# EI-CoreBioinformatics/portcullis

Measured on AMD Instinct MI355X. Metric: junc_reads_per_sec, higher is better.
Workload: dtype int32; 1 GPU; BASELINE configs[2]: synthetic 199999998 paired-end 150-bp reads, 25 contigs of GRCh38 lengths (3088286401 bp), 249999 junctions, orientation FR; reads_total=199999998, junctions_total=249999, contigs=25, reads_rank0=199999998, pairs_rank0=66692850

## Files before the change

portcullis_amd/csrc/pjb_api.hip:

```cpp
#include "pjb_host.hip.h"
#include "pjb_kernels.hip.h"

static int slot_init(pjb_ctx *c, int k);
static void aux_streams(pjb_ctx *c) {
    if (!c->stream3) (void)hipStreamCreateWithFlags(&c->stream3, hipStreamNonBlocking);
    if (!c->stream4) (void)hipStreamCreateWithFlags(&c->stream4, hipStreamNonBlocking);
}

extern "C" {

namespace {
std::mutex g_host_mu;
std::map<void *, size_t> g_host_registered;
}
void *pjb_host_alloc(size_t bytes) {
    if (bytes >= ((size_t)8 << 20)) {
        const size_t huge = (size_t)2 << 20, len = (bytes + huge - 1) & ~(huge - 1);
        void *p = mmap(nullptr, len, PROT_READ | PROT_WRITE, MAP_PRIVATE | MAP_ANONYMOUS, -1, 0);
        if (p != MAP_FAILED) {
            (void)madvise(p, len, MADV_HUGEPAGE);
            const size_t nt = std::min<size_t>(4, len >> 24);
            auto touch = [&](size_t t) {
                const size_t per = ((len / std::max<size_t>(nt, 1)) + huge - 1) & ~(huge - 1), a = std::min(len, per * t), b = std::min(len, a + per);
                for (size_t o = a; o < b; o += 4096) ((volatile uint8_t *)p)[o] = 0;
// ... 157 lines not shown
    extra_clear(c);
    for (auto &kv : c->filter_keys)
        if (kv.second.first) (void)hipFree(kv.second.first);
    c->filter_keys.clear();
    for (auto &g : c->contigs) free_contig(g);
    for (auto &b : c->genome_pool) release(b);
    c->genome_pool.clear();
    for (auto &sl : c->slab_pool)
        if (sl.p) (void)hipFree(sl.p);
    if (c->rows_pinned) (void)hipHostFree(c->rows_pinned);
    if (c->rows_table) (void)hipFree(c->rows_table);
    bam_stage_clear(c);
    for (int k = 0; k < PJB_MAX_QUEUED; k++) {
        CtlSlot &S = c->sl[k];
        if (S.pub) (void)hipHostFree(S.pub);
        if (S.batches_pinned) (void)hipHostFree(S.batches_pinned);
        for (auto &ev : S.ev)
            if (ev) (void)hipEventDestroy(ev);
        if (S.ev_rows) (void)hipEventDestroy(S.ev_rows);
        if (S.ev_done) (void)hipEventDestroy(S.ev_done);
        Buf *sb[] = {&S.x_q, &S.x_spos, &S.x_send, &S.x_gapoff, &S.x_zlist, &S.x_scnt, &S.x_codes, &S.cstats, &S.err, &S.gencount, &S.batches, &S.rows, &S.tile_cnt, &S.tile_stats, &S.splidx, &S.splpoff, &S.splrec, &S.tile_soff, &S.chunk_tile, &S.scan_parts, &S.members, &S.okey, &S.g,
                     &S.rec, &S.jidbam, &S.jkey, &S.total, &S.bitmap, &S.wrank, &S.pagecnt, &S.pagerank, &S.ends, &S.firstid,
                     &S.key[0], &S.key[1], &S.idx[0], &S.idx[1], &S.hist, &S.hist_scan, &S.hist_part, &S.bintotal, &S.scan_tiles, &S.jid, &S.seg, &S.runfirst,
                     &S.runstart, &S.ent, &S.entsum, &S.frag, &S.fragj, &S.masks, &S.acc, &S.ancl, &S.ancr, &S.genlist};
        for (Buf *b : sb) release(*b);
        hipEvent_t evs[] = {S.ev_k1, S.ev_xk1, S.ev_fork, S.ev_join, S.ev_fork2, S.ev_join2};
        for (hipEvent_t e : evs)
            if (e) (void)hipEventDestroy(e);
        if (S.main) (void)hipStreamDestroy(S.main);
        if (S.side) (void)hipStreamDestroy(S.side);
    }
    if (c->mirror_hdr) (void)hipHostFree(c->mirror_hdr);
    for (int k = 0; k < 2; k++) {
        if (c->stage[k]) (void)hipHostFree(c->stage[k]);
        if (c->stage_ev[k]) (void)hipEventDestroy(c->stage_ev[k]);
    }
    Buf *all[] = {&c->b_cursor, &c->b_scan_tiles, &c->b_hasx, &c->b_xtotal, &c->b_fasta_raw, &c->b_inf_comp, &c->b_inf_out, &c->b_inf_blocks, &c->b_inf_status, &c->b_inf_scratch, &c->b_inf_bitmap,
                  &c->b_bam_seg, &c->b_bam_rec, &c->b_bam_ctl, &c->f_pos, &c->f_cigoff, &c->f_cigar, &c->f_codes, &c->g_rows, &c->g_models, &c->g_refs,
                  &c->g_out, &c->g_bad,
                  &c->x_pos, &c->x_endx, &c->x_q, &c->x_prefq, &c->x_ce, &c->x_bound, &c->x_de, &c->x_dropped, &c->x_zlist, &c->x_cnt,
                  &c->x_tabk, &c->x_tabc, &c->x_rs, &c->x_re, &c->x_rr, &c->x_tileoff, &c->x_xrall, &c->x_tab,
                  &c->b_dfl_in, &c->b_dfl_sym, &c->b_dfl_slots, &c->b_dfl_size, &c->b_dfl_off, &c->b_dfl_packed};
    for (Buf *b : all) release(*b);
    for (auto &ch : c->xarena.chunks) (void)hipFree(ch.p);
    if (c->xrows_pinned) (void)hipHostFree(c->xrows_pinned);
    for (auto &pool : c->pools)
        for (auto &ev : pool.ev) (void)hipEventDestroy(ev);
// ... 590 lines not shown
        LAUNCH(c, "k4b_generic", k4b_generic, dim3(gen_grid), dim3(256), (const u64 *)S.genlist.p, (const u32 *)d_gen_cnt, gen_cap, (const u64 *)pr.key,
               pr.rec, (const u32 *)S.jidbam.p, kf, (const DevBatch *)S.batches.p, (int)batches.size(), (const int32_t *)S.ancl.p, (const int32_t *)S.ancr.p,
               GT, any_x ? 1 : 0, any_x ? 0 : 1, d_err, (const ContigStats *)d_cs, pack_nn, (const u32 *)S.splidx.p, (const uint4 *)S.splrec.p);
        return PJB_OK;
    };
    auto fork_k4b = [&]() -> int {
        if (!c->side_stream) return launch_k4b();
        HIP_TRY(c, hipEventRecord(S.ev_fork, st));
        HIP_TRY(c, hipStreamWaitEvent(S.side, S.ev_fork, 0));
        c->stream = S.side;
        f.forked = true;
        const int rc2 = launch_k4b();
        c->stream = st;
        if (rc2) return rc2;
        HIP_TRY(c, hipEventRecord(S.ev_join, S.side));
        return PJB_OK;
    };

    int sort_bits = kf.total_bits;
    const u32 rs_tiles = std::max<u32>(1, (PL + RS_TILE - 1) / RS_TILE);
    int n_pass = 1;
    std::vector<int> pass_bits;
    bool first_hist_done = false;
    auto plan_passes = [&]() -> int {
        n_pass = (sort_bits + c->radix_max_bits - 1) / c->radix_max_bits;
        if (n_pass < 1) n_pass = 1;
        pass_bits.assign((size_t)n_pass, sort_bits / n_pass);
        for (int p = 0; p < sort_bits % n_pass; p++) pass_bits[(size_t)p]++;
        const int dbits = pass_bits[0];
        int rc2;
        if ((rc2 = ensure(c, S.hist, (size_t)rs_tiles * (1u << dbits) * 4))) return rc2;
        if ((rc2 = ensure(c, S.hist_scan, (size_t)rs_tiles * (1u << dbits) * 4))) return rc2;
        if ((rc2 = ensure(c, S.bintotal, (size_t)4 << dbits))) return rc2;
        if ((rc2 = ensure(c, S.hist_part, (size_t)((rs_tiles + RSP_TILES - 1) / RSP_TILES) * (1u << dbits) * 4))) return rc2;
        return PJB_OK;
    };
    if (lim.dense) {
        const u32 cand_blocks = std::min<u32>(pair_blocks, 1024u);
        const u64 *okey = (const u64 *)pr.key;
        u64 *cand = (u64 *)S.key[1].p;
        const u32 n_pages = (u32)((n_words + ((size_t)1 << KD_PAGE_SHIFT) - 1) >> KD_PAGE_SHIFT);
        if ((rc = run_scan(c, "kd_rank", ArrU32Fn{(const u32 *)S.pagecnt.p}, ExclusiveU32Sink{(u32 *)S.pagerank.p}, (u64)n_pages, (u64 *)S.total.p)))
            return rc;
        LAUNCH(c, "kd_rank_pages", kd_rank_pages, dim3((n_pages + 3) / 4), dim3(256), (const u64 *)S.bitmap.p, (const u32 *)S.pagecnt.p, (const u32 *)S.pagerank.p,
               (u32 *)S.wrank.p, n_pages, (u32)n_words);
        u32 *cand_rank = (u32 *)S.idx[1].p;
        LAUNCH(c, "kd_ends", kd_ends, dim3(cand_blocks), dim3(256), (const u64 *)cand, kf, (const u64 *)S.bitmap.p, (const u32 *)S.wrank.p, JL,
               (u32 *)S.ends.p, cand_rank, d_cs);
        if ((rc = run_scan(c, "kd_first", EndsCountFn{(const u32 *)S.ends.p}, FirstIdSink{(u32 *)S.firstid.p, (int32_t *)S.ancl.p, (int32_t *)S.ancr.p},
                           (u64)JL, (u64 *)S.total.p)))
            return rc;
        LAUNCH(c, "kd_table", kd_table, dim3(cand_blocks), dim3(256), (const u64 *)cand, (const u64 *)S.ent.p, (const u32 *)cand_rank, kf, JL,
               (const u32 *)S.ends.p, (const u32 *)S.firstid.p, (const u64 *)S.total.p, (u64 *)S.jkey.p, (int32_t *)S.ancl.p, (int32_t *)S.ancr.p, d_cs,
               (const u32 *)d_gen_cnt, gen_cap, SL);
        sort_bits = std::max(1, bits_of((uint64_t)SL));
        if ((rc = plan_passes())) return rc;
        LAUNCH(c, "kd_assign", kd_assign, dim3(rs_tiles), dim3(256), okey, d_P, kf, (const u64 *)S.bitmap.p, (const u32 *)S.wrank.p,
               (const u32 *)S.ends.p, (const u32 *)S.firstid.p, JL, (const u64 *)S.total.p, (u32 *)S.jidbam.p, (u32 *)S.acc.p, (const u64 *)S.jkey.p,
               (const int32_t *)S.ancl.p, (const int32_t *)S.ancr.p, d_err, d_cs, pass_bits[0], (u32 *)S.hist.p);
        first_hist_done = true;
        if ((rc = fork_k4b())) return rc;
        LAUNCH(c, "kd_reset", kd_reset, dim3(cand_blocks), dim3(256), (const u64 *)cand, (const u32 *)cand_rank, kf, JL, (const ContigStats *)d_cs,
               (u64 *)S.bitmap.p, (u32 *)S.ends.p, (u32 *)S.pagecnt.p);
        S.dense_at_rest = true;
    } else if ((rc = plan_passes()))
        return rc;
    int cur = 0, shift = 0;
    auto sort_pass = [&](auto key_tag, const void *kin_v, void *kout_v, const u32 *vin, u32 *vout, int bits) -> int {
        using K = decltype(key_tag);
        const K *kin = (const K *)kin_v;
        K *kout = (K *)kout_v;
        if (!(shift == 0 && first_hist_done))
            LAUNCH(c, "rs_hist", rs_hist<K>, dim3(rs_tiles), dim3(256), kin, d_P, shift, bits, (u32 *)S.hist.p, rs_tiles);
        {
            const u32 nb = 1u << bits, n_panels = (rs_tiles + RSP_TILES - 1) / RSP_TILES;
            LAUNCH(c, "rs_panel_sums", rs_panel_sums, dim3(n_panels, (nb + 255) / 256), dim3(256), (const u32 *)S.hist.p, rs_tiles, nb, (u32 *)S.hist_part.p);
            LAUNCH(c, "rs_panel_scan", rs_panel_scan, dim3(n_panels, (nb + 255) / 256), dim3(256), (const u32 *)S.hist.p, (const u32 *)S.hist_part.p, rs_tiles, nb,
                   (u32 *)S.hist_scan.p, (u32 *)S.bintotal.p);
        }
#define RS_SCATTER(B)                                                                                                                          \
    LAUNCH_LDS(c, "rs_scatter", (rs_scatter<B, K>), dim3(rs_tiles), dim3(256), rs_scatter_lds_bytes(bits, sizeof(K)), kin, vin, kout, vout, d_P, \
               shift, bits, (const u32 *)S.hist_scan.p, (const u32 *)S.bintotal.p, rs_tiles)
        switch (bits) {
        case 9: RS_SCATTER(9); break;
        case 10: RS_SCATTER(10); break;
        case 11: RS_SCATTER(11); break;
        default: RS_SCATTER(0); break;
        }
#undef RS_SCATTER
        return PJB_OK;
    };
    for (int p = 0; p < n_pass; p++) {
        const int bits = pass_bits[(size_t)p];
        if (bits <= 0) break;
        const u32 *vin = p == 0 ? nullptr : (const u32 *)S.idx[cur].p;
        u32 *vout = (u32 *)S.idx[cur ^ 1].p;
        if (lim.dense) rc = sort_pass((u32)0, p == 0 ? S.jidbam.p : S.key[cur].p, S.key[cur ^ 1].p, vin, vout, bits);
        else rc = sort_pass((u64)0, p == 0 ? S.okey.p : S.key[cur].p, S.key[cur ^ 1].p, vin, vout, bits);
        if (rc) return rc;
        cur ^= 1;
        shift += bits;
    }
    f.n_pass = n_pass;
    const u32 *sidx = (const u32 *)S.idx[cur].p;
    f.sidx = sidx;
    const u32 *jid_sorted = lim.dense ? (const u32 *)S.key[cur].p : (const u32 *)S.jid.p;
    f.jid_sorted = jid_sorted;
    STAGE_EVENT(2);
    if ((rc = ensure(c, S.entsum, (size_t)JL * 8 + 16))) return rc;
    const u32 n_slices_lim = (PL + 63) / 64 + 1;
    const hipStream_t tl = st;
    auto entropy_kernels = [&]() -> int {
        LAUNCH(c, "k5_entropy_sum", k5_entropy_sum, dim3(std::max<u32>(1, (JL + 15) / 16)), dim3(256), (const u32 *)S.seg.p, (const u32 *)S.runfirst.p,
               (const u32 *)S.runstart.p, d_J, (double *)S.entsum.p);
        return PJB_OK;
    };
    bool entropy_forked = false;
    auto fork_entropy = [&]() -> int {
        if (!c->side_stream) return entropy_kernels();
        HIP_TRY(c, hipEventRecord(S.ev_fork2, st));
        HIP_TRY(c, hipStreamWaitEvent(S.side, S.ev_fork2, 0));
        c->stream = S.side;
        entropy_forked = true;
        const int rc2 = entropy_kernels();
// ... 168 lines not shown
            f.m_reads[m] += b.n;
            if (oc.last_known[k]) {
                prev_pos = oc.last_pos[k];
                prev_ptr = nullptr;
            } else
                prev_ptr = b.pos + (b.n - 1);
            b.member = (int32_t)m;
            f.batches.push_back(b);
            f.batch_member.push_back((int)m);
        }
    }
    f.tile_lo[f.tids.size()] = f.n_tiles;
    f.vlen = f.tids.size() > 1 ? at : c->ref_len[(size_t)f.tid];
    f.empty = f.batches.empty();
    ContigLimits &lim = f.lim;
    const u64 guess = std::min<u64>(0xffffff00ull, (u64)f.n_reads * 5 / 8 + 4096);
    lim.pair_limit = (u32)std::max<u64>(guess, 4096);
    lim.junc_limit = std::max<u32>(std::max<u32>(lim.pair_limit / 32, 4096), 2 * c->junc_seen * (u32)std::max<size_t>(1, f.tids.size() > 1 ? 2 : 1));
    if (!genomes_ok) lim.pair_limit = 0;
    lim.kf.raw = 0;
    lim.kf.lbits = std::max(1, c->lbits_seen);
    lim.kf.total_bits = lim.kf.lbits + std::max(1, bits_of((uint64_t)std::max<int64_t>(f.vlen, 1)));
    lim.dense = c->dense_ids;
    lim.sort_limit = c->junc_per_read > 0 ? std::min<u32>(lim.junc_limit, std::max<u32>(c->sort_floor, (u32)std::min<double>(4.0e9, 2.0 * c->junc_per_read * (double)f.n_reads + 64.0))) : 0u;
}

static int slot_init(pjb_ctx *c, int k) {
    CtlSlot &S = c->sl[k];
    if (S.ev_done) return PJB_OK;
    for (auto &ev : S.ev) HIP_TRY(c, hipEventCreate(&ev));
    HIP_TRY(c, hipEventCreateWithFlags(&S.ev_rows, hipEventDisableTiming));
    HIP_TRY(c, hipEventCreateWithFlags(&S.ev_done, hipEventDisableTiming));
    HIP_TRY(c, hipEventCreateWithFlags(&S.ev_k1, hipEventDisableTiming));
    HIP_TRY(c, hipEventCreateWithFlags(&S.ev_xk1, hipEventDisableTiming));
    HIP_TRY(c, hipEventCreateWithFlags(&S.ev_fork, hipEventDisableTiming));
    HIP_TRY(c, hipEventCreateWithFlags(&S.ev_join, hipEventDisableTiming));
    HIP_TRY(c, hipEventCreateWithFlags(&S.ev_fork2, hipEventDisableTiming));
    HIP_TRY(c, hipEventCreateWithFlags(&S.ev_join2, hipEventDisableTiming));
    HIP_TRY(c, hipStreamCreateWithFlags(&S.main, hipStreamNonBlocking));
    HIP_TRY(c, hipStreamCreateWithFlags(&S.side, hipStreamNonBlocking));
    return PJB_OK;
}

static int queue_chain(pjb_ctx *c, Flight &f) {
    int rc = queue_contig(c, f);
    if (!rc && c->extra) rc = extra_pre(c, f);
// ... 109 lines not shown
                                                  : "finish: more than 2^32 spliced pairs on one target are not supported");
            lim.pair_limit = (u32)cs.n_pairs + 64;
            lim.junc_limit = std::max<u32>(lim.junc_limit, lim.pair_limit / 8);
        }
        if (cs.overflow & OVF_KEYFMT) {
            const bool weird = cs.min_pos < 0 || cs.max_end > ref_len || cs.max_end < 0;
            if (weird && group) {
                *redo_single = true;
                return PJB_OK;
            }
            if (weird) {
                lim.kf.raw = 1;
                lim.kf.lbits = 32;
                lim.kf.total_bits = 64;
                lim.dense = false;
            } else {
                lim.kf.lbits = std::max(1, bits_of((uint64_t)cs.max_nlen));
                lim.kf.total_bits = lim.kf.lbits + std::max(1, bits_of((uint64_t)std::max(ref_len, 1)));
            }
        }
        const bool sort_only = (cs.overflow & OVF_JUNC) && lim.sort_limit && cs.n_junc <= lim.junc_limit;
        if (cs.overflow & OVF_JUNC) lim.sort_limit = 0;
        if ((cs.overflow & OVF_JUNC) && !sort_only) lim.junc_limit = std::max<u32>(cs.n_junc + 64, (cs.overflow & OVF_DENSE) || !lim.dense ? 0u : lim.junc_limit * 4);
        if (cs.overflow & OVF_DENSE) lim.dense = false;
        if (cs.overflow & OVF_LISTS) lim.list_cap = std::max(gen_list_cap(lim.pair_limit), (cs.list_need + cs.list_need / 4 + 511u) & ~255u);
    }
    if (c->extra && group) {
        bool apart = false;
        if ((rc = extra_group_apart(c, f, &apart))) return rc;
        if (apart) {
            unqueue_followers(c);
            if (f.forked) (void)hipStreamSynchronize(c->sl[f.slot].side);
            f.queued = f.forked = false;
            *redo_single = true;
            return PJB_OK;
        }
    }
    if (!lim.kf.raw) c->lbits_seen = std::max(c->lbits_seen, std::max(1, bits_of((uint64_t)cs.max_nlen)));
    const u32 P = cs.P, J = cs.J;
    pjb_region_result Rsum;
    memset(&Rsum, 0, sizeof Rsum);
    Rsum.min_len = INT32_MAX;
    if (!group) {
        pjb_region_result &R = res[0];
        R.spliced = cs.spliced;
        R.unspliced = cs.unspliced;
// ... 315 lines not shown
        if (b == std::string::npos) b = s.size();
        if (b > a) c->ktime_only.push_back(s.substr(a, b - a));
        a = b + 1;
    }
    return PJB_OK;
}

int pjb_reset_kernel_timing(pjb_ctx *c) {
    if (!c) return PJB_ERR_ARG;
    std::fill(c->kcount.begin(), c->kcount.end(), 0);
    std::fill(c->kms.begin(), c->kms.end(), 0.0);
    return PJB_OK;
}

int pjb_set_option(pjb_ctx *c, const char *name, int64_t value) {
    if (!c || !name) return PJB_ERR_ARG;
    if (c->n_fl) return fail(c, PJB_ERR_STATE, "set_option: target %d is still queued", c->fl[0].tid);
    const std::string n = name;
    if (n == "overlap") c->side_stream = value != 0;
    else if (n == "dense_ids") c->dense_ids = value != 0;
    else if (n == "extra_dense") c->extra_dense_only = value != 0;
    else if (n == "sort_floor") c->sort_floor = (u32)std::max<int64_t>(1, std::min<int64_t>(value, 1 << 30));
    else if (n == "window_skip") c->window_skip = value != 0;
    else if (n == "list_cap") c->list_cap_forced = (u32)std::max<int64_t>(0, std::min<int64_t>(value, 1 << 30));
    else return fail(c, PJB_ERR_ARG, "set_option: unknown option '%s'", name);
    return PJB_OK;
}

int pjb_get_timing(const pjb_ctx *c, pjb_timing *out) {
    if (!c || !out) return PJB_ERR_ARG;
    if (c->cfg.abi_version >= 4) *out = c->timing;
    else memcpy(out, &c->timing, offsetof(pjb_timing, repeats));
    return PJB_OK;
}

}
```

portcullis_amd/csrc/pjb_device.hip.h:

```cpp
#pragma once

#include <hip/hip_runtime.h>
#include <stdint.h>

#include "../../include/portcullis_amd.h"

namespace pjb {

typedef unsigned long long u64;
typedef unsigned int u32;

struct DevBatch {
    const int32_t *pos;
    const uint16_t *flag;
    const uint8_t *mapq;
    const uint8_t *xs;
    const int32_t *l_qseq;
    const int32_t *mtid;
    const int32_t *mpos;
    const uint32_t *cig_off;
    const uint32_t *cigar;
    const uint32_t *seq_off;
    const uint8_t *seq4;
    const u64 *name_hash;
// ... 2 lines not shown
    uint32_t tile_base;
    int32_t prev_pos;
    int32_t member;
    const int32_t *prev_pos_ptr;
    const uint32_t *seq2;
    const uint32_t *seq_exc;
};

__device__ inline void set_error(u64 *err, u32 ordinal, int code) {
    atomicMin(err, ((u64)ordinal << 8) | (u64)(u32)(-code));
}

struct TileStats {
    u32 spliced, unspliced;
    u64 sum_len;
    int32_t min_len, max_len;
    int32_t max_end;
    int32_t max_nlen;
    int32_t min_pos;
    u32 max_span;
};
static_assert(sizeof(TileStats) == 40, "TileStats layout");

enum : u32 { OVF_PAIRS = 1u, OVF_KEYFMT = 2u, OVF_JUNC = 4u, OVF_DENSE = 8u, OVF_LISTS = 16u };
struct ContigStats {
    u64 spliced, unspliced, sum_len;
    int32_t min_len, max_len;
    int32_t max_end, max_nlen, min_pos;
    u32 n_tiles;
    u64 n_pairs;
    u64 err;
    u32 n_junc, n_runs;
    u32 P;
    u32 J, R;
    u32 n_slots;
    u32 overflow;
    u32 n_cand;
    u32 n_slices;
    u32 list_need;
    u32 max_span;
};
static_assert(sizeof(ContigStats) == 112, "ContigStats layout");
__device__ __forceinline__ bool window_reach(u32 blk, u32 nl_prev, u32 nl_next, u32 B) {
    const u32 l = __builtin_elementwise_add_sat(blk, nl_prev), r = __builtin_elementwise_add_sat(__builtin_elementwise_add_sat(blk, nl_next), 1u);
    return l <= B || r <= B;
}

// ... 508 lines not shown
```

portcullis_amd/csrc/pjb_host.hip.h:

```cpp
#pragma once
#include "pjb_device.hip.h"
#include "pjb_extra_types.hip.h"

#include <algorithm>
#include <sys/mman.h>
#include <thread>
#include <chrono>
#include <cstdarg>
#include <cstdio>
#include <cstdlib>
#include <cstring>
#include <map>
#include <memory>
#include <mutex>
#include <string>
#include <thread>
#include <vector>

using namespace pjb;


inline thread_local std::string g_create_error;
inline thread_local std::string g_thread_error;
inline thread_local const void *g_thread_error_ctx = nullptr;
// ... 80 lines not shown
    u64 *spl_codes = nullptr;
    u32 n_spl = 0;
    bool dense = false;
    bool codes_in_table = false;
    SparseDepth sparse = {nullptr, nullptr, nullptr, nullptr, 0, 0, 0, 0};
    int32_t voff = 0;
};

struct XArena {
    struct Chunk {
        uint8_t *p;
        size_t cap;
    };
    std::vector<Chunk> chunks;
    size_t cur = 0, used = 0;
};

struct ContigLimits {
    u32 pair_limit = 0, junc_limit = 0;
    u32 list_cap = 0;
    u32 sort_limit = 0;
    KeyFmt kf;
    bool dense = false;
};

struct CtlSlot {
    Buf cstats, err, gencount, batches, rows;
    Buf x_q, x_spos, x_send, x_gapoff, x_zlist, x_scnt, x_codes;
    Buf tile_cnt, tile_stats, splidx, splpoff, splrec, tile_soff, chunk_tile;
    Buf scan_parts;
    u32 scan_epoch = 0;
    Buf members;
    Buf okey, rec, g, jidbam;
    hipEvent_t ev_k1 = nullptr;
    hipEvent_t ev_xk1 = nullptr;
    Buf total, bitmap, wrank, ends, firstid, key[2], idx[2], hist, hist_scan, hist_part, bintotal, scan_tiles;
    Buf pagecnt, pagerank;
    Buf jid, seg, runfirst, runstart, ent, entsum, frag, fragj, acc, ancl, ancr, jkey, genlist, masks;
    bool dense_at_rest = false;
    hipStream_t main = nullptr, side = nullptr;
    hipEvent_t ev_fork = nullptr, ev_join = nullptr, ev_fork2 = nullptr, ev_join2 = nullptr;
    uint8_t *pub = nullptr, *pub_dev = nullptr;
    DevBatch *batches_pinned = nullptr;
    size_t batches_pinned_cap = 0;
    bool at_rest = false;
    hipEvent_t ev[PJB_N_STAGES + 2] = {};
    hipEvent_t ev_rows = nullptr, ev_done = nullptr;
};
struct EvPool {
    std::vector<hipEvent_t> ev;
    size_t used = 0;
    std::vector<int> name;
};
constexpr int MISC_POOL = PJB_MAX_QUEUED;

struct Flight {
    int32_t tid = -1;
    std::vector<int32_t> tids;
    std::vector<int32_t> voff;
// ... 63 lines not shown
    pjb_junction_row *rows_table = nullptr;
    bool rows_copy_pending = false;
    int last_slot = 0;
    int inflate_lanes = 512 * 64;
    bool side_stream = true;
    bool dense_ids = true;
    u32 junc_seen = 0;
    int lbits_seen = 18;
    size_t rows_n = 0, rows_cap = 0;
    size_t rows_pinned_cap = 0;
    std::vector<void *> graveyard;
    std::mutex grave_mu;
    size_t last_rows_n = 0;
    uint8_t *mirror = nullptr;
    size_t mirror_cap = 0;
    int64_t *mirror_hdr = nullptr;
    size_t mirror_rows = 0;
    int64_t mirror_acc[5] = {0, 0, 0, INT32_MAX, 0};
    pjb_timing timing;
    int radix_max_bits = 11;
    double junc_per_read = 0;
    u32 sort_floor = 1u << 16;
    bool window_skip = true;
    u32 list_cap_forced = 0;
    bool k1_serial = true;
    hipEvent_t last_k1_ev = nullptr;
    int k1s_blocks_forced = 0;
    bool ktime = false;
    std::vector<std::string> knames;
    std::vector<int64_t> kcount;
    std::vector<double> kms;
    std::vector<std::string> ktime_only;
    Buf *scan_tiles = nullptr;
    Buf b_scan_tiles;
    Buf b_inf_comp, b_inf_out, b_inf_blocks, b_inf_status, b_inf_scratch, b_inf_bitmap;
    Buf b_dfl_in, b_dfl_sym, b_dfl_slots, b_dfl_size, b_dfl_off, b_dfl_packed;
    Buf b_bam_seg, b_bam_rec, b_bam_ctl;
    struct IndexState *index = nullptr;
    bool extra = false;
    std::vector<ExtraContig> xc;
    std::map<int32_t, std::pair<u64 *, u32>> filter_keys;
    Buf f_pos, f_cigoff, f_cigar, f_codes;
    Buf g_rows, g_models, g_refs, g_out, g_bad;
    Buf x_pos, x_endx, x_q, x_prefq, x_ce, x_bound, x_de, x_dropped, x_zlist, x_cnt, x_tabk, x_tabc, x_rs, x_re, x_rr, x_tileoff;
    Buf x_xrall, x_tab;
    size_t x_tab_slots = 0, x_tab_n = 0;
// ... 333 lines not shown
```

portcullis_amd/csrc/pjb_kernels.hip.h:

```cpp
#pragma once

#include "pjb_device.hip.h"

namespace pjb {

__global__ __launch_bounds__(256) void k0_upper(uint8_t *g, int64_t n, int do_upper, int *has_x) {
    int64_t i = ((int64_t)blockIdx.x * 256 + threadIdx.x) * 16;
    bool x = false;
    for (int64_t j = i; j < n && j < i + 16; j++) {
        uint8_t c = g[j];
        x |= (c == 'X' || (do_upper && c == 'x'));
    }
    if (__ballot(x) && lane_id() == 0) atomicOr(has_x, 1);
    if (!do_upper) return;
    if (i + 16 <= n && ((uintptr_t)(g + i) & 15) == 0) {
        uint4 v = *reinterpret_cast<uint4 *>(g + i);
        u32 *w = reinterpret_cast<u32 *>(&v);
#pragma unroll
        for (int k = 0; k < 4; k++) {
            u32 x = w[k], r = 0;
#pragma unroll
            for (int b = 0; b < 4; b++) {
                u32 c = (x >> (8 * b)) & 0xff;
                if (c >= 'a' && c <= 'z') c -= 32;
// ... 1879 lines not shown
    const uint4 a = q[0], b = q[1];
    return (a.x < ue) + (a.y < ue) + (a.z < ue) + (a.w < ue) + (b.x < ue) + (b.y < ue) + (b.z < ue) + (b.w < ue);
}
__device__ __forceinline__ void anchors_fold(bool valid, u32 j, int32_t l, int32_t r, int32_t *anc_l, int32_t *anc_r) {
    const u32 lk = (u32)l ^ 0x80000000u, rk = (u32)r ^ 0x80000000u;
    u64 todo = __ballot(valid);
    while (todo) {
        const int first = __ffsll((long long)todo) - 1;
        const u32 jc = (u32)__builtin_amdgcn_readlane((int)j, first);
        const bool mine = valid && j == jc;
        const u64 m = __ballot(mine);
        const int32_t lo = (int32_t)(wave_total<DppMin>(mine ? lk : 0xffffffffu) ^ 0x80000000u);
        const int32_t hi = (int32_t)(wave_total<DppMax>(mine ? rk : 0u) ^ 0x80000000u);
        if (lane_id() == first) {
            if (lo < __hip_atomic_load(&anc_l[jc], __ATOMIC_RELAXED, __HIP_MEMORY_SCOPE_AGENT)) atomicMin(&anc_l[jc], lo);
            if (hi > __hip_atomic_load(&anc_r[jc], __ATOMIC_RELAXED, __HIP_MEMORY_SCOPE_AGENT)) atomicMax(&anc_r[jc], hi);
        }
        todo &= ~m;
    }
}

__global__ __launch_bounds__(256) void kd_table(const u64 *cand, const u64 *cand_anc, const u32 *cand_rank, KeyFmt kf, u32 junc_limit, const u32 *ends,
                                                const u32 *first_id, const u64 *total, u64 *jkey, int32_t *anc_l, int32_t *anc_r, ContigStats *cs,
                                                const u32 *gen_cnt, u32 gen_cap, u32 sort_limit) {
    const u32 p = blockIdx.x * 256 + threadIdx.x;
    if (blockIdx.x == 0) {
        static_assert(GEN_SHARDS == 256, "a shard per thread of the first block");
        const u32 over = lists_over(gen_cnt, threadIdx.x, gen_cap);
        if (over) atomicMax(&cs->list_need, over);
        if (__syncthreads_or((int)over) && threadIdx.x == 0) cs->overflow |= OVF_LISTS;
    }
    if (p == 0) {
        const u64 J = *total;
        u32 ovf = cs->overflow;
        if (cs->P != 0 && (J > (u64)junc_limit || J > (u64)sort_limit)) {
            ovf |= OVF_JUNC;
            cs->overflow = ovf;
            cs->n_junc = (u32)(J < 0xffffffffull ? J : 0xffffffffull);
        }
        if (ovf) cs->P = 0;
        else if (cs->P) {
            const u32 n_pairs = cs->P;
            cs->n_junc = cs->J = (u32)J;
            cs->n_slices = (n_pairs + 63) / 64;
            cs->n_slots = (u32)J + (n_pairs + 63) / 64;
        }
    }
    const u32 n = cs->n_cand;
    for (u32 base = blockIdx.x * 256u; base < n; base += gridDim.x * 256u) {
        const u32 q = base + threadIdx.x;
        const bool on = q < n;
        const u32 pc = on ? q : n - 1;
        const u32 rs = cand_rank[pc];
        const u64 k = cand[pc], a = cand_anc[pc];
        bool valid = on && rs < junc_limit;
// ... 10 lines not shown
            if (lo < __hip_atomic_load(&anc_l[id], __ATOMIC_RELAXED, __HIP_MEMORY_SCOPE_AGENT)) atomicMin(&anc_l[id], lo);
            if (hi > __hip_atomic_load(&anc_r[id], __ATOMIC_RELAXED, __HIP_MEMORY_SCOPE_AGENT)) atomicMax(&anc_r[id], hi);
        }
    }
}

enum {
    F_N = 0, F_R1P, F_R1N, F_R2P, F_R2N, F_MS, F_XSP, F_XSN, F_UM, F_BPP, F_PPP, F_REL, F_DIST,
    F_MAXMINANC, F_UP, F_DOWN, F_MAXMMES, F_MAXMINMATCH,
    F_FIRSTMIS,
    F_PAD19,
    F_MISM_LO, F_MISM_HI,
    F_JAD0,
    F_WORDS = 48
};
__device__ __forceinline__ void acc_rest_state(u32 *acc, u64 n_junc) {
    const u64 n = n_junc * F_WORDS, step = (u64)gridDim.x * blockDim.x;
    for (u64 t = (u64)blockIdx.x * blockDim.x + threadIdx.x; t < n; t += step) acc[t] = (t % F_WORDS) == F_FIRSTMIS ? 100000000u : 0u;
}

constexpr int KDA_TILE = 4096;
__device__ __forceinline__ void wave_hist_add(u32 *h, u32 d, bool valid);
constexpr int KDA_PER = 4;
__global__ __launch_bounds__(256) void kd_assign(const u64 *key, const u32 *np, KeyFmt kf, const u64 *bitmap, const u32 *wrank, const u32 *ends,
                                                 const u32 *first_id, u32 junc_limit, const u64 *total, u32 *jid_bam, u32 *acc, const u64 *jkey,
                                                 const int32_t *anc_l, const int32_t *anc_r, u64 *err, ContigStats *cs_chk, int hist_bits, u32 *hist) {
    __shared__ u32 s_h[4096];
    const u32 n = *np;
    if (n == 0) {
        if (hist_bits > 0)
            for (u32 d = threadIdx.x; d < (1u << hist_bits); d += 256) hist[(size_t)blockIdx.x * (1u << hist_bits) + d] = 0;
        return;
    }
    {
        const u64 J = *total;
        acc_rest_state(acc, J < (u64)junc_limit ? J : (u64)junc_limit);
    }
    const u32 nb = hist_bits > 0 ? 1u << hist_bits : 0u;
    for (u32 d = threadIdx.x; d < nb; d += 256) s_h[d] = 0;
    if (nb) __syncthreads();
    for (u32 chunk = blockIdx.x * (KDA_TILE / (KDA_PER * 256)); chunk < (blockIdx.x + 1) * (KDA_TILE / (KDA_PER * 256)); chunk++) {
    if (chunk * (KDA_PER * 256) >= n) break;
    u64 kk[KDA_PER];
    u32 pp[KDA_PER];
#pragma unroll
    for (int q = 0; q < KDA_PER; q++) {
        pp[q] = (chunk * KDA_PER + q) * 256 + threadIdx.x;
        kk[q] = key[pp[q] < n ? pp[q] : n - 1];
    }
    bool lead[KDA_PER];
    int32_t ss[KDA_PER], ee[KDA_PER];
    u64 bw[KDA_PER];
    u32 wr[KDA_PER];
#pragma unroll
    for (int q = 0; q < KDA_PER; q++) {
        const u32 plo = (u32)__builtin_amdgcn_update_dpp(0, (int)(u32)kk[q], 0x138, 0xf, 0xf, false);
        const u32 phi = (u32)__builtin_amdgcn_update_dpp(0, (int)(u32)(kk[q] >> 32), 0x138, 0xf, 0xf, false);
        lead[q] = lane_id() == 0 || plo != (u32)kk[q] || phi != (u32)(kk[q] >> 32);
        unpack_key(kf, kk[q], ss[q], ee[q]);
        bw[q] = 0;
        wr[q] = 0;
        if (lead[q]) {
            bw[q] = bitmap[(u32)ss[q] >> 6];
            wr[q] = wrank[(u32)ss[q] >> 6];
        }
    }
    u32 rs_[KDA_PER], fi[KDA_PER], eb[KDA_PER];
#pragma unroll
    for (int q = 0; q < KDA_PER; q++) {
        rs_[q] = wr[q] + (u32)__popcll(bw[q] & ((1ull << (ss[q] & 63)) - 1ull));
        fi[q] = eb[q] = 0;
        if (lead[q]) {
            fi[q] = first_id[rs_[q]];
            eb[q] = ends_below(ends, rs_[q], (u32)ee[q]);
        }
    }
#pragma unroll
    for (int q = 0; q < KDA_PER; q++) {
        const u64 lm = __ballot(lead[q]) & ((2ull << lane_id()) - 1ull);
        const u32 id = (u32)__shfl((int)(fi[q] + eb[q]), 63 - __clzll((long long)lm), 64);
        fi[q] = id;
        eb[q] = 0;
        if (pp[q] < n) jid_bam[pp[q]] = id;
        if (nb) wave_hist_add(s_h, id & (nb - 1u), pp[q] < n);
    }
#ifdef PJB_SELFCHECK
    const u32 p = pp[0];
    if (p < n) {
    const int32_t s = ss[0], e = ee[0];
    const u32 rs = rs_[0], id = fi[0] + eb[0];
    {
        int bad = 0;
        const uint4 *q = reinterpret_cast<const uint4 *>(ends + (size_t)rs * DENSE_ENDS);
        const uint4 a = q[0], b = q[1];
        const u32 ue = (u32)e;
        if (!((bitmap[(u32)s >> 6] >> (s & 63)) & 1ull)) bad = 6;
        else if (!(a.x == ue || a.y == ue || a.z == ue || a.w == ue || b.x == ue || b.y == ue || b.z == ue || b.w == ue)) bad = 7;
        else if (id >= junc_limit || id >= (u32)*total) bad = 1;
        else if (jkey[id] != key[p]) bad = 2;
        else if (anc_l[id] > s || anc_r[id] < e) bad = 3;
        if (bad) {
            set_error(err, 0xfffff000u + (u32)bad, PJB_ERR_HIP);
            cs_chk->P = 0;
        }
    }
    }
#endif
    }
    if (nb) {
        __syncthreads();
        for (u32 d = threadIdx.x; d < nb; d += 256) hist[(size_t)blockIdx.x * nb + d] = s_h[d];
    }
}

constexpr int RS_ITEMS = 16;
constexpr int RS_TILE = 256 * RS_ITEMS;
constexpr int RS_MAX_BITS = 12;
constexpr int RS_MAX_BINS = 1 << RS_MAX_BITS;
static_assert(KDA_TILE == RS_TILE && RS_MAX_BINS <= 4096, "kd_assign counts the sort's first digit tile by tile");

__device__ __forceinline__ void wave_hist_add(u32 *h, u32 d, bool valid) {
    u64 rem = __ballot(valid);
    const int lane = lane_id();
#pragma unroll
    for (int it = 0; it < 2; it++) {
        if (rem == 0) return;
        const int first = __ffsll((long long)rem) - 1;
        const u32 d0 = __shfl(d, first, 64);
        const u64 m = __ballot(valid && d == d0) & rem;
        if (lane == first) atomicAdd(&h[d0], (u32)__popcll(m));
        rem &= ~m;
    }
    if ((rem >> lane) & 1ull) atomicAdd(&h[d], 1u);
}
// ... 183 lines not shown
    }
    __syncthreads();
    const u32 cnt = min((u32)RS_TILE, n - tile * RS_TILE);
    u32 digp[RS_ITEMS / 2];
#pragma unroll
    for (int r = 0; r < RS_ITEMS; r++) {
        const u32 j = r * 256 + threadIdx.x;
        const K kk = j < cnt ? kbuf[j] : (K)0;
        const u32 d = (u32)(kk >> shift) & mask;
        digp[r >> 1] = (r & 1) ? (digp[r >> 1] | (d << 16)) : d;
        if (j < cnt) kout[delta[d] + j] = kk;
    }
    __syncthreads();
#pragma unroll
    for (int r = 0; r < RS_ITEMS; r++) {
        const u32 i = base + r * 64 + lane;
        if (i < n) ibuf[(rkp[r >> 1] >> ((r & 1) * 16)) & 0xffffu] = val[r];
    }
    __syncthreads();
#pragma unroll
    for (int r = 0; r < RS_ITEMS; r++) {
        const u32 j = r * 256 + threadIdx.x;
        if (j < cnt) vout[delta[(digp[r >> 1] >> ((r & 1) * 16)) & 0xffffu] + j] = ibuf[j];
    }
}

struct HeadFn {
    const u64 *skey;
    const u32 *sidx;
    const PairRec *rec;
    __device__ u64 operator()(u64 i) const {
        const u64 im = i ? i - 1 : 0;
        const u64 ka = skey[i], kb = skey[im];
        const u32 sa = sidx[i], sb = sidx[im];
        const int32_t pa = rec[sa].pos, pb = rec[sb].pos;
        const bool hj = i == 0 || ka != kb;
        const bool hr = hj || pa != pb;
        return ((u64)hj << 32) | (u64)hr;
    }
};
struct HeadSink {
    u32 *jid_of;
    u32 *seg_off;
    u32 *run_first;
    u32 *run_start;
    const u64 *skey;
// ... 878 lines not shown
```

Baseline: 28.67 billion reads/s.

## Sort reads by junction via per-tile id runs instead of full radix sort

In dense mode, kd_assign now builds a per-tile histogram of junction ids within a bounded window and emits compact (id, tile) runs with counts. The runs, rather than all reads, are radix sorted, an exclusive scan over run counts gives destinations, and a new rs_place kernel scatters each read to its final sorted slot using wave-level ranking. This shrinks the sort input from one element per read to one per distinct id per tile. The cost is extra LDS work, a new overflow flag with fallback when a tile's id span exceeds the window or the run capacity is exceeded, and a stability requirement on the placement order.

```diff
diff --git a/portcullis_amd/csrc/pjb_api.hip b/portcullis_amd/csrc/pjb_api.hip
--- a/portcullis_amd/csrc/pjb_api.hip
+++ b/portcullis_amd/csrc/pjb_api.hip
@@ -203,7 +203,7 @@
         Buf *sb[] = {&S.x_q, &S.x_spos, &S.x_send, &S.x_gapoff, &S.x_zlist, &S.x_scnt, &S.x_codes, &S.cstats, &S.err, &S.gencount, &S.batches, &S.rows, &S.tile_cnt, &S.tile_stats, &S.splidx, &S.splpoff, &S.splrec, &S.tile_soff, &S.chunk_tile, &S.scan_parts, &S.members, &S.okey, &S.g,
                      &S.rec, &S.jidbam, &S.jkey, &S.total, &S.bitmap, &S.wrank, &S.pagecnt, &S.pagerank, &S.ends, &S.firstid,
                      &S.key[0], &S.key[1], &S.idx[0], &S.idx[1], &S.hist, &S.hist_scan, &S.hist_part, &S.bintotal, &S.scan_tiles, &S.jid, &S.seg, &S.runfirst,
-                     &S.runstart, &S.ent, &S.entsum, &S.frag, &S.fragj, &S.masks, &S.acc, &S.ancl, &S.ancr, &S.genlist};
+                     &S.runstart, &S.ent, &S.entsum, &S.frag, &S.fragj, &S.masks, &S.acc, &S.ancl, &S.ancr, &S.genlist, &S.runs};
         for (Buf *b : sb) release(*b);
         hipEvent_t evs[] = {S.ev_k1, S.ev_xk1, S.ev_fork, S.ev_join, S.ev_fork2, S.ev_join2};
         for (hipEvent_t e : evs)
@@ -840,6 +840,7 @@
     int n_pass = 1;
     std::vector<int> pass_bits;
     bool first_hist_done = false;
+    u32 plan_tiles = rs_tiles;
     auto plan_passes = [&]() -> int {
         n_pass = (sort_bits + c->radix_max_bits - 1) / c->radix_max_bits;
         if (n_pass < 1) n_pass = 1;
@@ -847,12 +848,42 @@
         for (int p = 0; p < sort_bits % n_pass; p++) pass_bits[(size_t)p]++;
         const int dbits = pass_bits[0];
         int rc2;
-        if ((rc2 = ensure(c, S.hist, (size_t)rs_tiles * (1u << dbits) * 4))) return rc2;
-        if ((rc2 = ensure(c, S.hist_scan, (size_t)rs_tiles * (1u << dbits) * 4))) return rc2;
+        if ((rc2 = ensure(c, S.hist, (size_t)plan_tiles * (1u << dbits) * 4))) return rc2;
+        if ((rc2 = ensure(c, S.hist_scan, (size_t)plan_tiles * (1u << dbits) * 4))) return rc2;
         if ((rc2 = ensure(c, S.bintotal, (size_t)4 << dbits))) return rc2;
-        if ((rc2 = ensure(c, S.hist_part, (size_t)((rs_tiles + RSP_TILES - 1) / RSP_TILES) * (1u << dbits) * 4))) return rc2;
+        if ((rc2 = ensure(c, S.hist_part, (size_t)((plan_tiles + RSP_TILES - 1) / RSP_TILES) * (1u << dbits) * 4))) return rc2;
         return PJB_OK;
     };
+    const bool run_route = lim.dense && lim.run_sort;
+    RunOut ro;
+    memset(&ro, 0, sizeof ro);
+    const u32 run_cap = (u32)std::min<u64>((u64)PL / 8 + 64ull * rs_tiles, 0xfff00000ull);
+    const u32 ro_tiles = (run_cap + RS_TILE - 1) / RS_TILE;
+    u64 *ro_total = nullptr, *ro_key[2] = {nullptr, nullptr};
+    u32 *run_dest = nullptr, *ro_idx[2] = {nullptr, nullptr};
+    if (run_route) {
+        auto al = [](size_t b) { return (b + 255) & ~(size_t)255; };
+        const size_t slack = (size_t)run_cap + RS_TILE;
+        const size_t at_tf = 256, at_tn = at_tf + al((size_t)rs_tiles * 4), at_key = at_tn + al((size_t)rs_tiles * 4), at_cnt = at_key + al(slack * 8),
+                     at_dest = at_cnt + al((size_t)run_cap * 4), at_k0 = at_dest + al((size_t)run_cap * 4), at_k1 = at_k0 + al(slack * 8),
+                     at_i0 = at_k1 + al(slack * 8), at_i1 = at_i0 + al(slack * 4), at_end = at_i1 + al(slack * 4);
+        if ((rc = ensure(c, S.runs, at_end))) return rc;
+        uint8_t *b = (uint8_t *)S.runs.p;
+        ro.n_runs = (u32 *)b;
+        ro_total = (u64 *)(b + 8);
+        ro.tile_first = (u32 *)(b + at_tf);
+        ro.tile_n = (u32 *)(b + at_tn);
+        ro.key = (u64 *)(b + at_key);
+        ro.cnt = (u32 *)(b + at_cnt);
+        run_dest = (u32 *)(b + at_dest);
+        ro_key[0] = (u64 *)(b + at_k0);
+        ro_key[1] = (u64 *)(b + at_k1);
+        ro_idx[0] = (u32 *)(b + at_i0);
+        ro_idx[1] = (u32 *)(b + at_i1);
+        ro.cap = run_cap;
+        ro.window = c->run_window ? std::min<u32>(c->run_window, RUN_W) : RUN_W;
+        ro.tile_bits = std::max(1, bits_of((uint64_t)rs_tiles));
+    }
     if (lim.dense) {
         const u32 cand_blocks = std::min<u32>(pair_blocks, 1024u);
         const u64 *okey = (const u64 *)pr.key;
@@ -870,13 +901,14 @@
             return rc;
         LAUNCH(c, "kd_table", kd_table, dim3(cand_blocks), dim3(256), (const u64 *)cand, (const u64 *)S.ent.p, (const u32 *)cand_rank, kf, JL,
                (const u32 *)S.ends.p, (const u32 *)S.firstid.p, (const u64 *)S.total.p, (u64 *)S.jkey.p, (int32_t *)S.ancl.p, (int32_t *)S.ancr.p, d_cs,
-               (const u32 *)d_gen_cnt, gen_cap, SL);
-        sort_bits = std::max(1, bits_of((uint64_t)SL));
+               (const u32 *)d_gen_cnt, gen_cap, SL, ro.n_runs);
+        sort_bits = std::max(1, bits_of((uint64_t)SL)) + (run_route ? ro.tile_bits : 0);
+        if (run_route) plan_tiles = ro_tiles;
         if ((rc = plan_passes())) return rc;
         LAUNCH(c, "kd_assign", kd_assign, dim3(rs_tiles), dim3(256), okey, d_P, kf, (const u64 *)S.bitmap.p, (const u32 *)S.wrank.p,
                (const u32 *)S.ends.p, (const u32 *)S.firstid.p, JL, (const u64 *)S.total.p, (u32 *)S.jidbam.p, (u32 *)S.acc.p, (const u64 *)S.jkey.p,
-               (const int32_t *)S.ancl.p, (const int32_t *)S.ancr.p, d_err, d_cs, pass_bits[0], (u32 *)S.hist.p);
-        first_hist_done = true;
+               (const int32_t *)S.ancl.p, (const int32_t *)S.ancr.p, d_err, d_cs, run_route ? 0 : pass_bits[0], (u32 *)S.hist.p, ro);
+        first_hist_done = !run_route;
         if ((rc = fork_k4b())) return rc;
         LAUNCH(c, "kd_reset", kd_reset, dim3(cand_blocks), dim3(256), (const u64 *)cand, (const u32 *)cand_rank, kf, JL, (const ContigStats *)d_cs,
                (u64 *)S.bitmap.p, (u32 *)S.ends.p, (u32 *)S.pagecnt.p);
@@ -884,21 +916,24 @@
     } else if ((rc = plan_passes()))
         return rc;
     int cur = 0, shift = 0;
-    auto sort_pass = [&](auto key_tag, const void *kin_v, void *kout_v, const u32 *vin, u32 *vout, int bits) -> int {
+    static const char *const rs_names[4] = {"rs_hist", "rs_panel_sums", "rs_panel_scan", "rs_scatter"};
+    static const char *const ro_names[6] = {"ro_hist", "ro_panel_sums", "ro_panel_scan", "ro_scatter", "ro_offsets", "rs_place"};
+    auto sort_pass = [&](auto key_tag, const void *kin_v, void *kout_v, const u32 *vin, u32 *vout, int bits, const u32 *d_n, u32 tiles,
+                         const char *const *names) -> int {
         using K = decltype(key_tag);
         const K *kin = (const K *)kin_v;
         K *kout = (K *)kout_v;
         if (!(shift == 0 && first_hist_done))
-            LAUNCH(c, "rs_hist", rs_hist<K>, dim3(rs_tiles), dim3(256), kin, d_P, shift, bits, (u32 *)S.hist.p, rs_tiles);
+            LAUNCH(c, names[0], rs_hist<K>, dim3(tiles), dim3(256), kin, d_n, shift, bits, (u32 *)S.hist.p, tiles);
         {
-            const u32 nb = 1u << bits, n_panels = (rs_tiles + RSP_TILES - 1) / RSP_TILES;
-            LAUNCH(c, "rs_panel_sums", rs_panel_sums, dim3(n_panels, (nb + 255) / 256), dim3(256), (const u32 *)S.hist.p, rs_tiles, nb, (u32 *)S.hist_part.p);
-            LAUNCH(c, "rs_panel_scan", rs_panel_scan, dim3(n_panels, (nb + 255) / 256), dim3(256), (const u32 *)S.hist.p, (const u32 *)S.hist_part.p, rs_tiles, nb,
+            const u32 nb = 1u << bits, n_panels = (tiles + RSP_TILES - 1) / RSP_TILES;
+            LAUNCH(c, names[1], rs_panel_sums, dim3(n_panels, (nb + 255) / 256), dim3(256), (const u32 *)S.hist.p, tiles, nb, (u32 *)S.hist_part.p);
+            LAUNCH(c, names[2], rs_panel_scan, dim3(n_panels, (nb + 255) / 256), dim3(256), (const u32 *)S.hist.p, (const u32 *)S.hist_part.p, tiles, nb,
                    (u32 *)S.hist_scan.p, (u32 *)S.bintotal.p);
         }
 #define RS_SCATTER(B)                                                                                                                          \
-    LAUNCH_LDS(c, "rs_scatter", (rs_scatter<B, K>), dim3(rs_tiles), dim3(256), rs_scatter_lds_bytes(bits, sizeof(K)), kin, vin, kout, vout, d_P, \
-               shift, bits, (const u32 *)S.hist_scan.p, (const u32 *)S.bintotal.p, rs_tiles)
+    LAUNCH_LDS(c, names[3], (rs_scatter<B, K>), dim3(tiles), dim3(256), rs_scatter_lds_bytes(bits, sizeof(K)), kin, vin, kout, vout, d_n, \
+               shift, bits, (const u32 *)S.hist_scan.p, (const u32 *)S.bintotal.p, tiles)
         switch (bits) {
         case 9: RS_SCATTER(9); break;
         case 10: RS_SCATTER(10); break;
@@ -911,13 +946,27 @@
     for (int p = 0; p < n_pass; p++) {
         const int bits = pass_bits[(size_t)p];
         if (bits <= 0) break;
-        const u32 *vin = p == 0 ? nullptr : (const u32 *)S.idx[cur].p;
-        u32 *vout = (u32 *)S.idx[cur ^ 1].p;
-        if (lim.dense) rc = sort_pass((u32)0, p == 0 ? S.jidbam.p : S.key[cur].p, S.key[cur ^ 1].p, vin, vout, bits);
-        else rc = sort_pass((u64)0, p == 0 ? S.okey.p : S.key[cur].p, S.key[cur ^ 1].p, vin, vout, bits);
+        if (run_route) {
+            rc = sort_pass((u64)0, p == 0 ? (const void *)ro.key : (const void *)ro_key[cur], ro_key[cur ^ 1], p == 0 ? nullptr : (const u32 *)ro_idx[cur],
+                           ro_idx[cur ^ 1], bits, (const u32 *)ro.n_runs, ro_tiles, ro_names);
+        } else {
+            const u32 *vin = p == 0 ? nullptr : (const u32 *)S.idx[cur].p;
+            u32 *vout = (u32 *)S.idx[cur ^ 1].p;
+            if (lim.dense) rc = sort_pass((u32)0, p == 0 ? S.jidbam.p : S.key[cur].p, S.key[cur ^ 1].p, vin, vout, bits, d_P, rs_tiles, rs_names);
+            else rc = sort_pass((u64)0, p == 0 ? S.okey.p : S.key[cur].p, S.key[cur ^ 1].p, vin, vout, bits, d_P, rs_tiles, rs_names);
+        }
         if (rc) return rc;
         cur ^= 1;
         shift += bits;
+    }
+    if (run_route) {
+        const u32 *order = ro_idx[cur];
+        if ((rc = run_scan(c, ro_names[4], RunCountFn{(const u32 *)ro.cnt, order}, RunDestSink{run_dest, order}, (u64)run_cap, ro_total, (const u32 *)ro.n_runs)))
+            return rc;
+        cur = 1;
+        LAUNCH(c, ro_names[5], rs_place, dim3(rs_tiles), dim3(256), (const u32 *)S.jidbam.p, d_P, (const u64 *)ro.key, (const u32 *)run_dest,
+               (const u32 *)ro.tile_first, (const u32 *)ro.tile_n, run_cap, ro.tile_bits, (u32 *)S.key[cur].p, (u32 *)S.idx[cur].p);
+        n_pass = 1;
     }
     f.n_pass = n_pass;
     const u32 *sidx = (const u32 *)S.idx[cur].p;
@@ -1132,6 +1181,7 @@
     lim.kf.lbits = std::max(1, c->lbits_seen);
     lim.kf.total_bits = lim.kf.lbits + std::max(1, bits_of((uint64_t)std::max<int64_t>(f.vlen, 1)));
     lim.dense = c->dense_ids;
+    lim.run_sort = c->run_sort;
     lim.sort_limit = c->junc_per_read > 0 ? std::min<u32>(lim.junc_limit, std::max<u32>(c->sort_floor, (u32)std::min<double>(4.0e9, 2.0 * c->junc_per_read * (double)f.n_reads + 64.0))) : 0u;
 }
 
@@ -1287,6 +1337,10 @@
         const bool sort_only = (cs.overflow & OVF_JUNC) && lim.sort_limit && cs.n_junc <= lim.junc_limit;
         if (cs.overflow & OVF_JUNC) lim.sort_limit = 0;
         if ((cs.overflow & OVF_JUNC) && !sort_only) lim.junc_limit = std::max<u32>(cs.n_junc + 64, (cs.overflow & OVF_DENSE) || !lim.dense ? 0u : lim.junc_limit * 4);
+        if (cs.overflow & OVF_RUNS) {
+            c->run_sort = false;
+            for (int k = 0; k < c->n_fl; k++) c->fl[k].lim.run_sort = false;
+        }
         if (cs.overflow & OVF_DENSE) lim.dense = false;
         if (cs.overflow & OVF_LISTS) lim.list_cap = std::max(gen_list_cap(lim.pair_limit), (cs.list_need + cs.list_need / 4 + 511u) & ~255u);
     }
@@ -1648,7 +1702,11 @@
     else if (n == "extra_dense") c->extra_dense_only = value != 0;
     else if (n == "sort_floor") c->sort_floor = (u32)std::max<int64_t>(1, std::min<int64_t>(value, 1 << 30));
     else if (n == "window_skip") c->window_skip = value != 0;
-    else if (n == "list_cap") c->list_cap_forced = (u32)std::max<int64_t>(0, std::min<int64_t>(value, 1 << 30));
+    else if (n == "run_sort") c->run_sort = value != 0;
+    else if (n == "run_window") {
+        if (value < 0 || value > (int64_t)RUN_W) return fail(c, PJB_ERR_ARG, "set_option: run_window takes 0 (the default, %u) to %u", RUN_W, RUN_W);
+        c->run_window = (u32)value;
+    } else if (n == "list_cap") c->list_cap_forced = (u32)std::max<int64_t>(0, std::min<int64_t>(value, 1 << 30));
     else return fail(c, PJB_ERR_ARG, "set_option: unknown option '%s'", name);
     return PJB_OK;
 }
diff --git a/portcullis_amd/csrc/pjb_device.hip.h b/portcullis_amd/csrc/pjb_device.hip.h
--- a/portcullis_amd/csrc/pjb_device.hip.h
+++ b/portcullis_amd/csrc/pjb_device.hip.h
@@ -48,7 +48,7 @@
 };
 static_assert(sizeof(TileStats) == 40, "TileStats layout");
 
-enum : u32 { OVF_PAIRS = 1u, OVF_KEYFMT = 2u, OVF_JUNC = 4u, OVF_DENSE = 8u, OVF_LISTS = 16u };
+enum : u32 { OVF_PAIRS = 1u, OVF_KEYFMT = 2u, OVF_JUNC = 4u, OVF_DENSE = 8u, OVF_LISTS = 16u, OVF_RUNS = 64u  };
 struct ContigStats {
     u64 spliced, unspliced, sum_len;
     int32_t min_len, max_len;
diff --git a/portcullis_amd/csrc/pjb_host.hip.h b/portcullis_amd/csrc/pjb_host.hip.h
--- a/portcullis_amd/csrc/pjb_host.hip.h
+++ b/portcullis_amd/csrc/pjb_host.hip.h
@@ -126,6 +126,7 @@
     u32 sort_limit = 0;
     KeyFmt kf;
     bool dense = false;
+    bool run_sort = false;
 };
 
 struct CtlSlot {
@@ -139,6 +140,7 @@
     hipEvent_t ev_k1 = nullptr;
     hipEvent_t ev_xk1 = nullptr;
     Buf total, bitmap, wrank, ends, firstid, key[2], idx[2], hist, hist_scan, hist_part, bintotal, scan_tiles;
+    Buf runs;
     Buf pagecnt, pagerank;
     Buf jid, seg, runfirst, runstart, ent, entsum, frag, fragj, acc, ancl, ancr, jkey, genlist, masks;
     bool dense_at_rest = false;
@@ -248,6 +250,8 @@
     double junc_per_read = 0;
     u32 sort_floor = 1u << 16;
     bool window_skip = true;
+    bool run_sort = true;
+    u32 run_window = 0;
     u32 list_cap_forced = 0;
     bool k1_serial = true;
     hipEvent_t last_k1_ev = nullptr;
diff --git a/portcullis_amd/csrc/pjb_kernels.hip.h b/portcullis_amd/csrc/pjb_kernels.hip.h
--- a/portcullis_amd/csrc/pjb_kernels.hip.h
+++ b/portcullis_amd/csrc/pjb_kernels.hip.h
@@ -1925,7 +1925,7 @@
 
 __global__ __launch_bounds__(256) void kd_table(const u64 *cand, const u64 *cand_anc, const u32 *cand_rank, KeyFmt kf, u32 junc_limit, const u32 *ends,
                                                 const u32 *first_id, const u64 *total, u64 *jkey, int32_t *anc_l, int32_t *anc_r, ContigStats *cs,
-                                                const u32 *gen_cnt, u32 gen_cap, u32 sort_limit) {
+                                                const u32 *gen_cnt, u32 gen_cap, u32 sort_limit, u32 *n_runs) {
     const u32 p = blockIdx.x * 256 + threadIdx.x;
     if (blockIdx.x == 0) {
         static_assert(GEN_SHARDS == 256, "a shard per thread of the first block");
@@ -1934,6 +1934,7 @@
         if (__syncthreads_or((int)over) && threadIdx.x == 0) cs->overflow |= OVF_LISTS;
     }
     if (p == 0) {
+        if (n_runs) *n_runs = 0;
         const u64 J = *total;
         u32 ovf = cs->overflow;
         if (cs->P != 0 && (J > (u64)junc_limit || J > (u64)sort_limit)) {
@@ -1990,10 +1991,32 @@
 constexpr int KDA_TILE = 4096;
 __device__ __forceinline__ void wave_hist_add(u32 *h, u32 d, bool valid);
 constexpr int KDA_PER = 4;
+constexpr u32 RUN_W = 2048;
+struct RunOut {
+    u64 *key;
+    u32 *cnt;
+    u32 *tile_first;
+    u32 *tile_n;
+    u32 *n_runs;
+    u32 cap;
+    u32 window;
+    int tile_bits;
+};
+static_assert(RUN_W == 256 * 8, "kd_assign compacts eight table entries a thread");
+__device__ __forceinline__ void runs_close_chain(ContigStats *cs) {
+    atomicOr(&cs->overflow, OVF_RUNS);
+    cs->P = 0;
+    cs->J = 0;
+    cs->n_slots = 0;
+    cs->n_slices = 0;
+}
 __global__ __launch_bounds__(256) void kd_assign(const u64 *key, const u32 *np, KeyFmt kf, const u64 *bitmap, const u32 *wrank, const u32 *ends,
                                                  const u32 *first_id, u32 junc_limit, const u64 *total, u32 *jid_bam, u32 *acc, const u64 *jkey,
-                                                 const int32_t *anc_l, const int32_t *anc_r, u64 *err, ContigStats *cs_chk, int hist_bits, u32 *hist) {
+                                                 const int32_t *anc_l, const int32_t *anc_r, u64 *err, ContigStats *cs_chk, int hist_bits, u32 *hist,
+                                                 RunOut ro) {
     __shared__ u32 s_h[4096];
+    __shared__ u32 s_run[4];
+    __shared__ u32 s_rscan[4];
     const u32 n = *np;
     if (n == 0) {
         if (hist_bits > 0)
@@ -2005,8 +2028,13 @@
         acc_rest_state(acc, J < (u64)junc_limit ? J : (u64)junc_limit);
     }
     const u32 nb = hist_bits > 0 ? 1u << hist_bits : 0u;
-    for (u32 d = threadIdx.x; d < nb; d += 256) s_h[d] = 0;
-    if (nb) __syncthreads();
+    for (u32 d = threadIdx.x; d < (ro.window ? RUN_W : nb); d += 256) s_h[d] = 0;
+    if (threadIdx.x == 0) {
+        s_run[0] = 0xffffffffu;
+        s_run[1] = 0u;
+    }
+    if (nb || ro.window) __syncthreads();
+    u32 id_lo = 0xffffffffu, id_hi = 0u;
     for (u32 chunk = blockIdx.x * (KDA_TILE / (KDA_PER * 256)); chunk < (blockIdx.x + 1) * (KDA_TILE / (KDA_PER * 256)); chunk++) {
     if (chunk * (KDA_PER * 256) >= n) break;
     u64 kk[KDA_PER];
@@ -2051,6 +2079,13 @@
         eb[q] = 0;
         if (pp[q] < n) jid_bam[pp[q]] = id;
         if (nb) wave_hist_add(s_h, id & (nb - 1u), pp[q] < n);
+        if (ro.window) {
+            wave_hist_add(s_h, id & (RUN_W - 1u), pp[q] < n);
+            if (pp[q] < n) {
+                id_lo = id < id_lo ? id : id_lo;
+                id_hi = id > id_hi ? id : id_hi;
+            }
+        }
     }
 #ifdef PJB_SELFCHECK
     const u32 p = pp[0];
@@ -2078,6 +2113,59 @@
     if (nb) {
         __syncthreads();
         for (u32 d = threadIdx.x; d < nb; d += 256) hist[(size_t)blockIdx.x * nb + d] = s_h[d];
+    }
+    if (ro.window) {
+        id_lo = wave_total<DppMin>(id_lo);
+        id_hi = wave_total<DppMax>(id_hi);
+        if (lane_id() == 0) {
+            atomicMin(&s_run[0], id_lo);
+            atomicMax(&s_run[1], id_hi);
+        }
+        __syncthreads();
+        const u32 lo = s_run[0], hi = s_run[1];
+        if (lo > hi) {
+            if (threadIdx.x == 0) ro.tile_n[blockIdx.x] = 0;
+            return;
+        }
+        if (hi - lo >= ro.window) {
+            if (threadIdx.x == 0) {
+                ro.tile_n[blockIdx.x] = 0;
+                runs_close_chain(cs_chk);
+            }
+            return;
+        }
+        const u32 span = hi - lo + 1u;
+        u32 c[8], nz = 0;
+#pragma unroll
+        for (int k = 0; k < 8; k++) {
+            const u32 o = threadIdx.x * 8u + (u32)k;
+            c[k] = o < span ? s_h[(lo + o) & (RUN_W - 1u)] : 0u;
+            nz += c[k] != 0u;
+        }
+        u32 tot;
+        u32 at = block_escan_256<u32>(nz, s_rscan, &tot);
+        if (threadIdx.x == 0) {
+            u32 b = atomicAdd(ro.n_runs, tot);
+            if (b > ro.cap || tot > ro.cap - b) {
+                atomicSub(ro.n_runs, tot);
+                b = 0xffffffffu;
+                runs_close_chain(cs_chk);
+            }
+            s_run[2] = b;
+            ro.tile_first[blockIdx.x] = b == 0xffffffffu ? 0u : b;
+            ro.tile_n[blockIdx.x] = b == 0xffffffffu ? 0u : tot;
+        }
+        __syncthreads();
+        const u32 first = s_run[2];
+        if (first == 0xffffffffu) return;
+        at += first;
+#pragma unroll
+        for (int k = 0; k < 8; k++)
+            if (c[k]) {
+                ro.key[at] = ((u64)(lo + threadIdx.x * 8u + (u32)k) << ro.tile_bits) | (u64)blockIdx.x;
+                ro.cnt[at] = c[k];
+                at++;
+            }
     }
 }
 
@@ -2307,6 +2395,71 @@
     for (int r = 0; r < RS_ITEMS; r++) {
         const u32 j = r * 256 + threadIdx.x;
         if (j < cnt) vout[delta[(digp[r >> 1] >> ((r & 1) * 16)) & 0xffffu] + j] = ibuf[j];
+    }
+}
+
+struct RunCountFn {
+    const u32 *cnt, *order;
+    __device__ u64 operator()(u64 i) const { return cnt[order[i]]; }
+};
+struct RunDestSink {
+    u32 *dest;
+    const u32 *order;
+    __device__ void operator()(u64 i, u64, u64 ex) const { dest[order[i]] = (u32)ex; }
+};
+__global__ __launch_bounds__(256) void rs_place(const u32 *jid_bam, const u32 *np, const u64 *run_key, const u32 *run_dest, const u32 *tile_first,
+                                                const u32 *tile_n, u32 run_cap, int tile_bits, u32 *kout, u32 *vout) {
+    __shared__ u32 s_dest[RUN_W];
+    __shared__ unsigned short s_wcnt[4][RUN_W];
+    const u32 n = *np;
+    const u32 tile = blockIdx.x;
+    if ((u64)tile * RS_TILE >= n) return;
+    for (u32 d = threadIdx.x; d < 2 * RUN_W; d += 256) ((u32 *)&s_wcnt[0][0])[d] = 0;
+    const u32 tf = tile_first[tile], tn = tf < run_cap ? min(tile_n[tile], min(RUN_W, run_cap - tf)) : 0u;
+    for (u32 e = threadIdx.x; e < tn; e += 256) s_dest[(u32)(run_key[tf + e] >> tile_bits) & (RUN_W - 1u)] = run_dest[tf + e];
+    const int w = __builtin_amdgcn_readfirstlane(threadIdx.x >> 6), lane = lane_id();
+    unsigned short *wc = s_wcnt[w];
+    const u32 base = tile * RS_TILE + w * (RS_TILE / 4);
+    const u64 lt = (1ull << lane) - 1;
+    u32 id[RS_ITEMS];
+    u32 rkp[RS_ITEMS / 2];
+    const u32 *kp = jid_bam + base;
+#pragma unroll
+    for (int r = 0; r < RS_ITEMS; r++) id[r] = kp[r * 64 + lane];
+    __syncthreads();
+#pragma unroll
+    for (int r = 0; r < RS_ITEMS; r++) {
+        const bool valid = base + r * 64 + lane < n;
+        const u32 d = id[r] & (RUN_W - 1u);
+        u32 rank = 0;
+        u64 todo = __ballot(valid);
+        while (todo) {
+            const int first = __ffsll((long long)todo) - 1;
+            const u32 idc = (u32)__builtin_amdgcn_readlane((int)id[r], first);
+            const bool mine = valid && id[r] == idc;
+            const u64 m = __ballot(mine);
+            u32 before = 0;
+            if (lane == first) {
+                before = wc[d];
+                wc[d] = (unsigned short)(before + (u32)__popcll(m));
+            }
+            before = (u32)__builtin_amdgcn_readlane((int)before, first);
+            if (mine) rank = before + (u32)__popcll(m & lt);
+            todo &= ~m;
+        }
+        rkp[r >> 1] = (r & 1) ? (rkp[r >> 1] | (rank << 16)) : rank;
+    }
+    __syncthreads();
+#pragma unroll
+    for (int r = 0; r < RS_ITEMS; r++) {
+        const u32 i = base + r * 64 + lane;
+        const u32 d = id[r] & (RUN_W - 1u);
+        u32 dst = s_dest[d] + ((rkp[r >> 1] >> ((r & 1) * 16)) & 0xffffu);
+        for (int q = 0; q < w; q++) dst += s_wcnt[q][d];
+        if (i < n && dst < n) {
+            kout[dst] = id[r];
+            vout[dst] = i;
+        }
     }
 }
 
```

Result: faster. 29.49 billion reads/s, median of 6 (+2.9%).
